# Linyou/Ced-NeRF

Measured on NVIDIA B200. Metric: train_step_rays_per_s, higher is better.
Workload: dtype f16 (MLP, tables) / f32 (marching, compositing, grads)

## Files before the change

cednerf_b200/csrc/march.cu:

```cuda
#include "common.cuh"

#define MARCH_MAX_LEVELS 8

namespace {

struct MarchArgs {
  const float* rays_o;
  const float* rays_d;
  int64_t n_rays;
  const uint32_t* occ_bits;
  const float* aabbs;
  int n_levels;
  int res;
  const float* near;
  const float* far;
  float near_const, far_const;
  float step_size, cone_angle;
  int limit;
  const uint8_t* mask;
  const float* t_sorted;
  const int64_t* t_indices;
  const uint8_t* hits;
  const int64_t* iv_starts;
  const int64_t* sm_starts;
  float* iv_vals;
  uint8_t* iv_left;
  uint8_t* iv_right;
  int64_t* iv_ray;
  float* sm_vals;
  int64_t* sm_ray;
  uint8_t* sm_valid;
  float* t_starts;
  float* t_ends;
  int64_t* ray_indices;
  int32_t* n_intervals;
  int32_t* n_samples;
  float* termination;
  float* run_t;
  int32_t* run_n;
  int32_t* n_runs;
  int run_cap;
  const int32_t* order;
  const int32_t* n_active_dev;
  const int32_t* limit_dev;
  int by_slot;
  const uint32_t* coarse;
};

__device__ __forceinline__ float clampf(float v, float lo, float hi) { return fminf(fmaxf(v, lo), hi); }
__device__ __forceinline__ int clampi(int v, int lo, int hi) { return v < lo ? lo : (v > hi ? hi : v); }
__device__ __forceinline__ float step_dt(float t, float cone, float step) { return clampf(t * cone, step, 1e10f); }

__device__ __forceinline__ void advance_to(float& t_last, float t_target, float cone, float step_size) {
  if (step_size <= 0.0f) {
    t_last = t_target;
    return;
  }
  if (cone == 0.0f && step_size <= 1e10f && t_last == t_last && t_last - t_last == 0.0f) {
    const float half = step_size * 0.5f;
    while (t_last + half < t_target) t_last += step_size;
    return;
  }
  while (!(t_last * cone >= step_size && t_target * cone < 1e10f)) {
    const float dt = step_dt(t_last, cone, step_size);
    if (t_last + dt * 0.5f >= t_target) return;
    t_last += dt;
  }
  float t = t_last;
  for (;;) {
    const float d0 = t * cone;
    const float t1 = t + d0, d1 = t1 * cone;
    const float t2 = t1 + d1, d2 = t2 * cone;
    const float t3 = t2 + d2, d3 = t3 * cone;
    const bool e0 = t + d0 * 0.5f >= t_target, e1 = t1 + d1 * 0.5f >= t_target;
    const bool e2 = t2 + d2 * 0.5f >= t_target, e3 = t3 + d3 * 0.5f >= t_target;
    if (e0 | e1 | e2 | e3) {
      t_last = e0 ? t : (e1 ? t1 : (e2 ? t2 : t3));
      return;
    }
    t = t3 + d3;
  }
}

__device__ __forceinline__ void slab(const float* o, const float* inv, const float* bx, float near, float far,
                                     float miss, float& t_min, float& t_max, bool& hit) {
  float tmin = -INFINITY, tmax = INFINITY;
#pragma unroll
  for (int a = 0; a < 3; ++a) {
    const float t1 = (bx[a] - o[a]) * inv[a];
    const float t2 = (bx[3 + a] - o[a]) * inv[a];
    tmin = fmaxf(tmin, fminf(t1, t2));
    tmax = fminf(tmax, fmaxf(t1, t2));
  }
  hit = (tmax > tmin) && (tmax > 0.0f);
  t_min = hit ? clampf(tmin, near, far) : miss;
  t_max = hit ? clampf(tmax, near, far) : miss;
}

__global__ void ray_aabb_kernel(const float* __restrict__ rays_o, const float* __restrict__ rays_d, int64_t n,
                                const float* __restrict__ aabbs, int L, float near, float far, float miss,
                                float* __restrict__ t_mins, float* __restrict__ t_maxs, uint8_t* __restrict__ hits) {
  const int64_t r = (int64_t)blockIdx.x * blockDim.x + threadIdx.x;
  if (r >= n) return;
  const float o[3] = {rays_o[3 * r], rays_o[3 * r + 1], rays_o[3 * r + 2]};
  const float inv[3] = {1.0f / rays_d[3 * r], 1.0f / rays_d[3 * r + 1], 1.0f / rays_d[3 * r + 2]};
  for (int l = 0; l < L; ++l) {
    float a, b;
    bool h;
    slab(o, inv, aabbs + 6 * l, near, far, miss, a, b, h);
    t_mins[r * L + l] = a;
    t_maxs[r * L + l] = b;
    hits[r * L + l] = (uint8_t)h;
  }
}

__device__ __forceinline__ void sort_bounds(float* v, int* id, int m) {
  for (int i = 1; i < m; ++i) {
    const float kv = v[i];
    const int ki = id[i];
    int j = i - 1;
    while (j >= 0 && v[j] > kv) {
      v[j + 1] = v[j];
      id[j + 1] = id[j];
      --j;
    }
    v[j + 1] = kv;
    id[j + 1] = ki;
  }
}

__global__ void sort_boundaries_kernel(const float* __restrict__ t_mins, const float* __restrict__ t_maxs, int64_t n,
                                       int L, float* __restrict__ t_sorted, int64_t* __restrict__ t_indices) {
  const int64_t r = (int64_t)blockIdx.x * blockDim.x + threadIdx.x;
  if (r >= n) return;
  float v[2 * MARCH_MAX_LEVELS];
  int id[2 * MARCH_MAX_LEVELS];
  const int m = 2 * L;
  for (int l = 0; l < L; ++l) {
    v[l] = t_mins[r * L + l];
    v[L + l] = t_maxs[r * L + l];
  }
  for (int i = 0; i < m; ++i) id[i] = i;
  sort_bounds(v, id, m);
  for (int i = 0; i < m; ++i) {
    t_sorted[r * m + i] = v[i];
    t_indices[r * m + i] = id[i];
  }
}

#ifndef MARCH_MIN_BLOCKS
#define MARCH_MIN_BLOCKS 6
#endif
template <bool FILL, bool COARSE = false>
__global__ void __launch_bounds__(128, MARCH_MIN_BLOCKS) march_kernel(MarchArgs a) {
  const int64_t slot = (int64_t)blockIdx.x * blockDim.x + threadIdx.x;
  if (slot >= a.n_rays) return;
  if (a.n_active_dev && slot >= (int64_t)*a.n_active_dev) {
    if (!FILL && a.n_samples) a.n_samples[slot] = 0;
    if (!FILL && a.n_runs) a.n_runs[slot] = 0;
    return;
  }
  const int64_t r = a.order ? (int64_t)a.order[slot] : slot;
  const int64_t oi = a.by_slot ? slot : r;
  const float near = a.near ? a.near[r] : a.near_const;
  const float far = a.far ? a.far[r] : a.far_const;
  if (a.mask && !a.mask[oi]) {
    if (a.n_intervals) a.n_intervals[oi] = 0;
    if (a.n_samples) a.n_samples[oi] = 0;
    if (a.termination && !(FILL && a.by_slot)) a.termination[r] = near;
    if (!FILL && a.n_runs) a.n_runs[oi] = 0;
    return;
  }
  const int L = a.n_levels, m = 2 * L, res = a.res;
  const float eps = 1e-6f;
  const float o[3] = {a.rays_o[3 * r], a.rays_o[3 * r + 1], a.rays_o[3 * r + 2]};
  const float d[3] = {a.rays_d[3 * r], a.rays_d[3 * r + 1], a.rays_d[3 * r + 2]};
  const float inv[3] = {1.0f / d[0], 1.0f / d[1], 1.0f / d[2]};
  const float fres = (float)res;
  const int64_t cells_per_level = (int64_t)res * res * res;

  float ts[2 * MARCH_MAX_LEVELS];
  int ti[2 * MARCH_MAX_LEVELS];
  bool hit[MARCH_MAX_LEVELS];
  if (a.t_sorted) {
    for (int i = 0; i < m; ++i) {
      ts[i] = a.t_sorted[r * m + i];
      ti[i] = (int)a.t_indices[r * m + i];
    }
    for (int l = 0; l < L; ++l) hit[l] = a.hits[r * L + l] != 0;
  } else {
    for (int l = 0; l < L; ++l) slab(o, inv, a.aabbs + 6 * l, -INFINITY, INFINITY, INFINITY, ts[l], ts[L + l], hit[l]);
    for (int i = 0; i < m; ++i) ti[i] = i;
    sort_bounds(ts, ti, m);
  }

  const int64_t iv_base = FILL && a.iv_starts ? a.iv_starts[oi] : 0;
  const int64_t sm_base = FILL && a.sm_starts ? a.sm_starts[oi] : 0;
  int n_iv = 0, n_sm = 0;
  float t_last = near;
  int continuous = 0;
  int runs = 0, run_len = 0;
  const int limit = a.limit_dev ? *a.limit_dev : a.limit;
  const float step_size = a.step_size, cone = a.cone_angle;

  for (int i = 0; i < m - 1; ++i) {
    const int bi = ti[i];
    const bool entering = bi < L;
    int level = bi % L;
    if (!hit[level]) continue;
    if (!entering) {
      const int bn = ti[i + 1];
      if (bn < L) continue;
      level = bn % L;
      if (!hit[level]) continue;
    }
    const float this_tmin = fmaxf(ts[i], near);
    const float this_tmax = fminf(ts[i + 1], far);
    if (this_tmin >= this_tmax) continue;

    if (!continuous) advance_to(t_last, this_tmin, cone, step_size);

    const float* bx = a.aabbs + 6 * level;
    float tdist[3], delta[3];
    int cur[3], overflow[3], stepi[3];
    const float tstart = this_tmin + eps, tend = this_tmax - eps;
#pragma unroll
    for (int ax = 0; ax < 3; ++ax) {
      const float extent = bx[3 + ax] - bx[ax];
      const float voxel = extent / fres;
      const float start = o[ax] + d[ax] * tstart;
      const float end = o[ax] + d[ax] * tend;
      int c = (int)(((start - bx[ax]) / extent) * fres);
      int f = (int)(((end - bx[ax]) / extent) * fres);
      c = clampi(c, 0, res - 1);
      f = clampi(f, 0, res - 1);
      const int start_idx = c + (d[ax] > 0.0f ? 1 : 0);
      const float tmax_a = ((bx[ax] + (((float)start_idx * voxel) - start)) * inv[ax]) + this_tmin;
      const float stepf = (d[ax] == 0.0f) ? 0.0f : (d[ax] > 0.0f ? 1.0f : -1.0f);
      tdist[ax] = (d[ax] == 0.0f) ? this_tmax : tmax_a;
      delta[ax] = (d[ax] == 0.0f) ? this_tmax : (voxel * inv[ax]) * stepf;
      stepi[ax] = (int)stepf;
      cur[ax] = c;
      overflow[ax] = f + stepi[ax];
    }

    float t_pend = 0.0f;
    int pend = 0;
    int eb0 = -1, eb1 = -1, eb2 = -1;
    auto catch_up = [&](float t_target) { advance_to(t_last, t_target, cone, step_size); };
    uint32_t cell = ((uint32_t)cur[0] * (uint32_t)res + (uint32_t)cur[1]) * (uint32_t)res + (uint32_t)cur[2] +
                    (uint32_t)level * (uint32_t)cells_per_level;
    int dcell[3] = {stepi[0] * res * res, stepi[1] * res, stepi[2]};
    asm volatile("" : "+r"(dcell[0]), "+r"(dcell[1]));
    while (limit <= 0 || n_sm < limit) {
      const float t_trav = fminf(fminf(tdist[0], fminf(tdist[1], tdist[2])), this_tmax);
      bool occupied = false;
      if (!(COARSE && (cur[0] >> 2) == eb0 && (cur[1] >> 2) == eb1 && (cur[2] >> 2) == eb2)) {
        occupied = (__ldg(a.occ_bits + (cell >> 5)) >> (cell & 31u)) & 1u;
        if (COARSE && !occupied) {
          const int cres = res >> 2;
          const int64_t cb = ((int64_t)(cur[0] >> 2) * cres + (cur[1] >> 2)) * cres + (cur[2] >> 2) +
                             (int64_t)level * cres * cres * cres;
          const bool block_occupied = (__ldg(a.coarse + (cb >> 5)) >> (cb & 31)) & 1u;
          eb0 = block_occupied ? -1 : (cur[0] >> 2);
          eb1 = cur[1] >> 2;
          eb2 = cur[2] >> 2;
        }
      }
      if (!occupied) {
        t_pend = t_trav;
        pend = 1;
        continuous = 0;
      } else {
        if (pend) {
          catch_up(t_pend);
          pend = 0;
        }
        while (limit <= 0 || n_sm < limit) {
          float t_next;
          if (step_size <= 0.0f) {
            t_next = t_trav;
          } else {
            const float dt = step_dt(t_last, cone, step_size);
            if (t_last + dt * 0.5f >= t_trav) break;
            t_next = t_last + dt;
          }
          if (FILL) {
            if (a.iv_vals) {
              const int64_t k = iv_base + n_iv;
              if (!continuous) {
                a.iv_vals[k] = t_last;
                a.iv_ray[k] = r;
                a.iv_left[k] = 1;
                a.iv_vals[k + 1] = t_next;
                a.iv_ray[k + 1] = r;
                a.iv_right[k + 1] = 1;
              } else {
                a.iv_vals[k] = t_next;
                a.iv_ray[k] = r;
                a.iv_left[k - 1] = 1;
                a.iv_right[k] = 1;
              }
            }
            const int64_t k = sm_base + n_sm;
            if (a.sm_vals) {
              a.sm_vals[k] = (t_next + t_last) * 0.5f;
              a.sm_ray[k] = r;
              a.sm_valid[k] = 1;
            }
            if (a.t_starts) {
              a.t_starts[k] = t_last;
              a.t_ends[k] = t_next;
              a.ray_indices[k] = r;
            }
          }
          if (!FILL && a.run_t) {
            if (!continuous) {
              if (runs > 0 && runs <= a.run_cap) a.run_n[oi * a.run_cap + runs - 1] = run_len;
              if (runs < a.run_cap) a.run_t[oi * a.run_cap + runs] = t_last;
              ++runs;
              run_len = 0;
            }
            ++run_len;
          }
          n_iv += continuous ? 1 : 2;
          n_sm += 1;
          continuous = 1;
          t_last = t_next;
          if (t_next >= t_trav) break;
        }
      }
      const bool s0 = tdist[0] < tdist[1] && tdist[0] < tdist[2];
      const bool s1 = !s0 && tdist[1] < tdist[2];
      const bool s2 = !s0 && !s1;
      const float n0 = tdist[0] + delta[0], n1 = tdist[1] + delta[1], n2 = tdist[2] + delta[2];
      tdist[0] = s0 ? n0 : tdist[0];
      tdist[1] = s1 ? n1 : tdist[1];
      tdist[2] = s2 ? n2 : tdist[2];
      cur[0] += s0 ? stepi[0] : 0;
      cur[1] += s1 ? stepi[1] : 0;
      cur[2] += s2 ? stepi[2] : 0;
      cell += (uint32_t)(s0 ? dcell[0] : (s1 ? dcell[1] : dcell[2]));
      const bool done = (s0 & (cur[0] == overflow[0])) | (s1 & (cur[1] == overflow[1])) | (s2 & (cur[2] == overflow[2]));
      if (done) break;
    }
    if (pend) catch_up(t_pend);
  }
  if (!FILL && a.run_t) {
    if (runs > 0 && runs <= a.run_cap) a.run_n[oi * a.run_cap + runs - 1] = run_len;
    a.n_runs[oi] = runs;
  }
  if (a.n_intervals) a.n_intervals[oi] = n_iv;
  if (a.n_samples) a.n_samples[oi] = n_sm;
  const bool refilled = a.by_slot && !FILL && runs > a.run_cap;
  if (a.termination && !refilled) a.termination[r] = t_last;
}

__global__ void __launch_bounds__(128)
march_fill_runs_kernel(int64_t n_rays, const int64_t* __restrict__ sm_starts, const float* __restrict__ run_t,
                       const int32_t* __restrict__ run_n, const int32_t* __restrict__ n_runs, int run_cap,
                       float step_size, float cone, float* __restrict__ t_starts, float* __restrict__ t_ends,
                       int64_t* __restrict__ ray_indices, uint8_t* __restrict__ overflow,
                       const int32_t* __restrict__ capped_counts, const int32_t* __restrict__ slot_ray = nullptr,
                       const int32_t* __restrict__ n_active_dev = nullptr) {
  const int64_t r = (int64_t)blockIdx.x * blockDim.x + threadIdx.x;
  if (r >= n_rays) return;
  if (n_active_dev && r >= (int64_t)*n_active_dev) {
    overflow[r] = 0;
    return;
  }
  const int64_t ray_id = slot_ray ? (int64_t)slot_ray[r] : r;
  const int runs = n_runs[r];
  bool over = runs > run_cap;
  int64_t k = sm_starts[r];
  const int64_t k_end = capped_counts ? sm_starts[r + 1] : INT64_MAX;
  if (capped_counts && over && k_end - k != (int64_t)capped_counts[r]) {
    for (; k < k_end; ++k) t_starts[k] = 0.0f, t_ends[k] = 0.0f, ray_indices[k] = ray_id;
    over = false;
    overflow[r] = 0;
    return;
  }
  overflow[r] = (uint8_t)over;
  if (over) return;
  auto next = [&](float t) { return (step_size <= 0.0f) ? t : t + step_dt(t, cone, step_size); };
  for (int j = 0; j < runs; ++j) {
    float t = run_t[r * run_cap + j];
    int cnt = run_n[r * run_cap + j];
    if ((int64_t)cnt > k_end - k) cnt = (int)(k_end - k);
    int i = 0;
    for (; i < cnt && (k & 3); ++i, ++k) {
      const float t_next = next(t);
      t_starts[k] = t, t_ends[k] = t_next, ray_indices[k] = ray_id;
      t = t_next;
    }
    for (; i + 4 <= cnt; i += 4, k += 4) {
      const float a1 = next(t), a2 = next(a1), a3 = next(a2), a4 = next(a3);
      *reinterpret_cast<float4*>(t_starts + k) = make_float4(t, a1, a2, a3);
      *reinterpret_cast<float4*>(t_ends + k) = make_float4(a1, a2, a3, a4);
      const longlong2 rr = make_longlong2((long long)ray_id, (long long)ray_id);
      *reinterpret_cast<longlong2*>(ray_indices + k) = rr;
      *reinterpret_cast<longlong2*>(ray_indices + k + 2) = rr;
      t = a4;
    }
    for (; i < cnt; ++i, ++k) {
      const float t_next = next(t);
      t_starts[k] = t, t_ends[k] = t_next, ray_indices[k] = ray_id;
      t = t_next;
    }
  }
}

__global__ void pack_bits_kernel(const uint8_t* __restrict__ bin, int64_t n_cells, uint32_t* __restrict__ bits) {
  const int64_t i = (int64_t)blockIdx.x * blockDim.x + threadIdx.x;
  const bool b = i < n_cells && bin[i] != 0;
  const unsigned w = __ballot_sync(0xffffffffu, b);
  if ((threadIdx.x & 31) == 0 && i < n_cells) bits[i >> 5] = w;
}

__global__ void occ_threshold_kernel(const float* __restrict__ occs, int64_t n_cells, const float* __restrict__ thre,
                                     uint8_t* __restrict__ bin, uint32_t* __restrict__ bits) {
  const int64_t i = (int64_t)blockIdx.x * blockDim.x + threadIdx.x;
// ... 132 lines not shown
      totals[0] = t < capacity ? t : capacity;
      totals[1] = t;
    }
  }
  __syncthreads();
  int64_t off = excl_s + local;
#pragma unroll
  for (int k = 0; k < SCAN_ITEMS; ++k) {
    if (base + k < n) offsets[base + k] = off < capacity ? off : capacity;
    off += c[k];
  }
}

}

CEDNERF_EXPORT int cednerf_ray_aabb_intersect(const float* rays_o, const float* rays_d, int64_t n_rays,
                                              const float* aabbs, int n_levels, float near_plane, float far_plane,
                                              float miss_value, float* t_mins, float* t_maxs, uint8_t* hits,
                                              void* stream) {
  CEDNERF_REQUIRE(n_rays >= 0 && n_levels >= 1, "bad sizes");
  if (n_rays == 0) return 0;
  ray_aabb_kernel<<<cednerf_blocks(n_rays, 256), 256, 0, (cudaStream_t)stream>>>(
      rays_o, rays_d, n_rays, aabbs, n_levels, near_plane, far_plane, miss_value, t_mins, t_maxs, hits);
  return cednerf_check_launch("cednerf_ray_aabb_intersect");
}

CEDNERF_EXPORT int cednerf_sort_boundaries(const float* t_mins, const float* t_maxs, int64_t n_rays, int n_levels,
                                           float* t_sorted, int64_t* t_indices, void* stream) {
  CEDNERF_REQUIRE(n_rays >= 0 && n_levels >= 1 && n_levels <= MARCH_MAX_LEVELS, "bad sizes (levels <= 8)");
  if (n_rays == 0) return 0;
  sort_boundaries_kernel<<<cednerf_blocks(n_rays, 256), 256, 0, (cudaStream_t)stream>>>(t_mins, t_maxs, n_rays,
                                                                                       n_levels, t_sorted, t_indices);
  return cednerf_check_launch("cednerf_sort_boundaries");
}

CEDNERF_EXPORT int cednerf_occ_pack_bits(const uint8_t* binaries, int64_t n_cells, uint32_t* bits, void* stream) {
  CEDNERF_REQUIRE(n_cells > 0, "empty grid");
  pack_bits_kernel<<<cednerf_blocks(n_cells, 256), 256, 0, (cudaStream_t)stream>>>(binaries, n_cells, bits);
  return cednerf_check_launch("cednerf_occ_pack_bits");
}

CEDNERF_EXPORT int cednerf_occ_threshold_pack(const float* occs, int64_t n_cells, const float* threshold_dev,
                                              uint8_t* binaries, uint32_t* bits, void* stream) {
  CEDNERF_REQUIRE(n_cells > 0 && (n_cells % 32) == 0, "cell count must be a multiple of 32");
  occ_threshold_kernel<<<cednerf_blocks(n_cells, 256), 256, 0, (cudaStream_t)stream>>>(occs, n_cells, threshold_dev,
                                                                                      binaries, bits);
  return cednerf_check_launch("cednerf_occ_threshold_pack");
}

namespace {

__global__ void __launch_bounds__(256) occ_mark_invisible_kernel(const float* __restrict__ K, int n_K,
                                                                 const float* __restrict__ c2w, int n_cams, int c2w_rows,
                                                                 const float* __restrict__ aabbs, int res,
                                                                 int64_t cells_per_level, int64_t n_cells, float width,
                                                                 float height, float near, float* __restrict__ occs) {
  __shared__ float cam[64][21];
  const int64_t cell = (int64_t)blockIdx.x * blockDim.x + threadIdx.x;
  const bool active = cell < n_cells;
  float xw[3] = {0.f, 0.f, 0.f};
  if (active) {
    const int level = (int)(cell / cells_per_level);
    const int64_t c = cell - (int64_t)level * cells_per_level;
    const int coord[3] = {(int)(c / ((int64_t)res * res)), (int)((c / res) % res), (int)(c % res)};
    const float* bx = aabbs + 6 * level;
#pragma unroll
    for (int k = 0; k < 3; ++k) {
      const float x01 = __fdiv_rn((float)coord[k], (float)(res - 1));
      xw[k] = __fadd_rn(bx[k], __fmul_rn(x01, __fsub_rn(bx[3 + k], bx[k])));
    }
  }
  bool covered = false, too_near = false;
  for (int c0 = 0; c0 < n_cams; c0 += 64) {
    const int nc = n_cams - c0 < 64 ? n_cams - c0 : 64;
    __syncthreads();
    for (int q = threadIdx.x; q < nc; q += blockDim.x) {
      const float* m = c2w + (int64_t)(c0 + q) * c2w_rows * 4;
      const float* k = K + (n_K == 1 ? 0 : (int64_t)(c0 + q) * 9);
      float* d = cam[q];
#pragma unroll
      for (int i = 0; i < 3; ++i) {
#pragma unroll
        for (int j = 0; j < 3; ++j) d[3 * i + j] = m[4 * j + i];
        d[9 + i] = -__fadd_rn(__fadd_rn(__fmul_rn(m[i], m[3]), __fmul_rn(m[4 + i], m[7])), __fmul_rn(m[8 + i], m[11]));
      }
#pragma unroll
      for (int j = 0; j < 9; ++j) d[12 + j] = k[j];
    }
    __syncthreads();
    if (active) {
      for (int q = 0; q < nc; ++q) {
        const float* d = cam[q];
        float xc[3], uvd[3];
#pragma unroll
        for (int i = 0; i < 3; ++i)
          xc[i] = __fadd_rn(__fadd_rn(__fadd_rn(__fmul_rn(d[3 * i], xw[0]), __fmul_rn(d[3 * i + 1], xw[1])),
                                      __fmul_rn(d[3 * i + 2], xw[2])),
                            d[9 + i]);
#pragma unroll
        for (int i = 0; i < 3; ++i)
          uvd[i] = __fadd_rn(__fadd_rn(__fmul_rn(d[12 + 3 * i], xc[0]), __fmul_rn(d[12 + 3 * i + 1], xc[1])),
                             __fmul_rn(d[12 + 3 * i + 2], xc[2]));
        const float u = __fdiv_rn(uvd[0], uvd[2]), v = __fdiv_rn(uvd[1], uvd[2]);
        const bool in_image = uvd[2] >= 0.f && u >= 0.f && u < width && v >= 0.f && v < height;
        covered = covered || (uvd[2] >= near && in_image);
        too_near = too_near || (uvd[2] < near && in_image);
      }
    }
  }
  if (active) occs[cell] = (covered && !too_near) ? 0.f : -1.f;
}

}

CEDNERF_EXPORT int cednerf_occ_mark_invisible(const float* K, int n_K, const float* c2w, int n_cams, int c2w_rows,
                                              const float* aabbs, int n_levels, int resolution, int width, int height,
                                              float near_plane, float* occs, void* stream) {
  CEDNERF_REQUIRE(K && c2w && aabbs && occs, "null argument");
  CEDNERF_REQUIRE(n_cams >= 1 && (n_K == 1 || n_K == n_cams) && (c2w_rows == 3 || c2w_rows == 4), "bad camera arrays");
  CEDNERF_REQUIRE(n_levels >= 1 && resolution >= 2, "bad grid");
  const int64_t cpl = (int64_t)resolution * resolution * resolution, n_cells = cpl * n_levels;
  occ_mark_invisible_kernel<<<cednerf_blocks(n_cells, 256), 256, 0, (cudaStream_t)stream>>>(
      K, n_K, c2w, n_cams, c2w_rows, aabbs, resolution, cpl, n_cells, (float)width, (float)height, near_plane, occs);
  return cednerf_check_launch("cednerf_occ_mark_invisible");
}

namespace {

__global__ void ray_coherence_keys_kernel(const float* __restrict__ rays_d, int64_t n, int32_t* __restrict__ keys) {
  const int64_t r = (int64_t)blockIdx.x * blockDim.x + threadIdx.x;
  if (r >= n) return;
  const float x = rays_d[3 * r], y = rays_d[3 * r + 1], z = rays_d[3 * r + 2];
  const float inv = 1.0f / fmaxf(fabsf(x) + fabsf(y) + fabsf(z), 1e-20f);
  float u = x * inv, v = y * inv;
  if (z < 0.0f) {
    const float fu = (1.0f - fabsf(v)) * (u >= 0.0f ? 1.0f : -1.0f), fv = (1.0f - fabsf(u)) * (v >= 0.0f ? 1.0f : -1.0f);
    u = fu, v = fv;
  }
  uint32_t qu = (uint32_t)fminf(fmaxf((u * 0.5f + 0.5f) * 1023.0f, 0.0f), 1023.0f);
  uint32_t qv = (uint32_t)fminf(fmaxf((v * 0.5f + 0.5f) * 1023.0f, 0.0f), 1023.0f);
  auto spread = [](uint32_t b) {
    b = (b | (b << 8)) & 0x00ff00ffu;
    b = (b | (b << 4)) & 0x0f0f0f0fu;
    b = (b | (b << 2)) & 0x33333333u;
    b = (b | (b << 1)) & 0x55555555u;
    return b;
  };
  keys[r] = (int32_t)(spread(qu) | (spread(qv) << 1));
}

__global__ void occ_coarsen_kernel(const uint32_t* __restrict__ bits, int n_levels, int res, uint32_t* __restrict__ coarse) {
  const int cres = res >> 2;
  const int64_t per_level = (int64_t)cres * cres * cres, total = per_level * n_levels;
  const int64_t i = (int64_t)blockIdx.x * blockDim.x + threadIdx.x;
  if (i * 32 >= total) return;
  uint32_t w = 0u;
  for (int j = 0; j < 32; ++j) {
    const int64_t cb = i * 32 + j;
    if (cb >= total) break;
    const int level = (int)(cb / per_level);
    const int64_t r = cb - level * per_level;
    const int bz = (int)(r % cres), by = (int)((r / cres) % cres), bx = (int)(r / ((int64_t)cres * cres));
    bool any = false;
    for (int dx = 0; dx < 4 && !any; ++dx)
      for (int dy = 0; dy < 4 && !any; ++dy) {
        const int64_t c0 = ((int64_t)(4 * bx + dx) * res + (4 * by + dy)) * res + 4 * bz + (int64_t)level * res * res * res;
        for (int dz = 0; dz < 4; ++dz) {
          const int64_t c = c0 + dz;
          any = any || ((bits[c >> 5] >> (c & 31)) & 1u);
        }
      }
    if (any) w |= 1u << j;
  }
  coarse[i] = w;
}

#define ORDER_BINS 16384
__global__ void order_hist_kernel(const int32_t* __restrict__ keys, int64_t n, uint32_t* __restrict__ hist) {
  const int64_t i = (int64_t)blockIdx.x * blockDim.x + threadIdx.x;
  if (i < n) atomicAdd(hist + (((uint32_t)keys[i]) >> 6), 1u);
}
__global__ void __launch_bounds__(1024) order_scan_kernel(uint32_t* __restrict__ hist) {
  __shared__ uint32_t warp_tot[32];
  uint32_t v[16], s = 0;
#pragma unroll
  for (int k = 0; k < 16; ++k) v[k] = hist[threadIdx.x * 16 + k], s += v[k];
  uint32_t incl = s;
  const int lane = threadIdx.x & 31, warp = threadIdx.x >> 5;
#pragma unroll
  for (int o = 1; o < 32; o <<= 1) {
    const uint32_t t = __shfl_up_sync(0xffffffffu, incl, o);
    if (lane >= o) incl += t;
  }
  if (lane == 31) warp_tot[warp] = incl;
  __syncthreads();
  if (warp == 0) {
    uint32_t w = warp_tot[lane], wi = w;
#pragma unroll
    for (int o = 1; o < 32; o <<= 1) {
      const uint32_t t = __shfl_up_sync(0xffffffffu, wi, o);
      if (lane >= o) wi += t;
    }
    warp_tot[lane] = wi - w;
  }
  __syncthreads();
  uint32_t off = warp_tot[warp] + incl - s;
#pragma unroll
  for (int k = 0; k < 16; ++k) hist[threadIdx.x * 16 + k] = off, off += v[k];
}
__global__ void order_scatter_kernel(const int32_t* __restrict__ keys, int64_t n, uint32_t* __restrict__ cursor,
                                     int32_t* __restrict__ order) {
  const int64_t i = (int64_t)blockIdx.x * blockDim.x + threadIdx.x;
  if (i < n) order[atomicAdd(cursor + (((uint32_t)keys[i]) >> 6), 1u)] = (int32_t)i;
}

}

CEDNERF_EXPORT int cednerf_ray_coherence_order(const int32_t* keys, int64_t n_rays, int32_t* order, void* workspace,
                                               void* stream) {
  CEDNERF_REQUIRE(n_rays >= 0 && n_rays < (1ll << 31) && keys && order && workspace, "bad arguments");
  if (n_rays == 0) return 0;
  cudaStream_t st = (cudaStream_t)stream;
  uint32_t* hist = (uint32_t*)workspace;
  cudaMemsetAsync(hist, 0, ORDER_BINS * sizeof(uint32_t), st);
  order_hist_kernel<<<cednerf_blocks(n_rays, 256), 256, 0, st>>>(keys, n_rays, hist);
  order_scan_kernel<<<1, 1024, 0, st>>>(hist);
  order_scatter_kernel<<<cednerf_blocks(n_rays, 256), 256, 0, st>>>(keys, n_rays, hist, order);
  return cednerf_check_launch("cednerf_ray_coherence_order", 3);
}

CEDNERF_EXPORT int cednerf_occ_coarsen(const uint32_t* occ_bits, int n_levels, int resolution, uint32_t* coarse, void* stream) {
  CEDNERF_REQUIRE(occ_bits && coarse && n_levels >= 1 && resolution >= 4 && resolution % 4 == 0, "bad arguments");
  const int cres = resolution / 4;
  const int64_t words = ((int64_t)cres * cres * cres * n_levels + 31) / 32;
  occ_coarsen_kernel<<<cednerf_blocks(words, 128), 128, 0, (cudaStream_t)stream>>>(occ_bits, n_levels, resolution, coarse);
  return cednerf_check_launch("cednerf_occ_coarsen");
}

CEDNERF_EXPORT int cednerf_ray_coherence_keys(const float* rays_d, int64_t n_rays, int32_t* keys, void* stream) {
  CEDNERF_REQUIRE(n_rays >= 0 && rays_d && keys, "bad arguments");
  if (n_rays == 0) return 0;
  ray_coherence_keys_kernel<<<cednerf_blocks(n_rays, 256), 256, 0, (cudaStream_t)stream>>>(rays_d, n_rays, keys);
  return cednerf_check_launch("cednerf_ray_coherence_keys");
}

CEDNERF_EXPORT int cednerf_march(int fill, const float* rays_o, const float* rays_d, int64_t n_rays,
                                 const uint32_t* occ_bits, const float* aabbs, int n_levels, int resolution,
                                 const float* near_planes, const float* far_planes, float near_const, float far_const,
                                 float step_size, float cone_angle, int steps_limit, const uint8_t* rays_mask,
                                 const float* t_sorted, const int64_t* t_indices, const uint8_t* hits,
                                 const int64_t* iv_starts, const int64_t* sm_starts, float* iv_vals, uint8_t* iv_left,
                                 uint8_t* iv_right, int64_t* iv_ray, float* sm_vals, int64_t* sm_ray,
                                 uint8_t* sm_valid, float* t_starts, float* t_ends, int64_t* ray_indices,
                                 int32_t* n_intervals, int32_t* n_samples, float* termination, float* run_t,
                                 int32_t* run_n, int32_t* n_runs, int run_cap, const int32_t* ray_order,
                                 const uint32_t* occ_coarse, void* stream) {
  CEDNERF_REQUIRE(!run_t || (!fill && run_n && n_runs && run_cap > 0 && step_size > 0.0f),
                  "run recording: count pass, positive step size");
  CEDNERF_REQUIRE((int64_t)n_levels * resolution * resolution * resolution < (1ll << 31), "occupancy grid too large");
  CEDNERF_REQUIRE(n_rays >= 0 && n_levels >= 1 && n_levels <= MARCH_MAX_LEVELS && resolution >= 1,
                  "bad sizes (levels <= 8)");
  CEDNERF_REQUIRE((t_sorted == nullptr) == (t_indices == nullptr) && (t_sorted == nullptr) == (hits == nullptr),
                  "t_sorted, t_indices and hits go together");
  CEDNERF_REQUIRE(!fill || ((!t_starts && !sm_vals) || sm_starts) , "fill pass needs sm_starts");
  CEDNERF_REQUIRE(!fill || !iv_vals || iv_starts, "fill pass needs iv_starts");
  CEDNERF_REQUIRE(!t_starts || (t_ends && ray_indices), "packed outputs go together");
  if (n_rays == 0) return 0;
  MarchArgs a{rays_o, rays_d, n_rays, occ_bits, aabbs, n_levels, resolution, near_planes, far_planes, near_const,
              far_const, step_size, cone_angle, steps_limit, rays_mask, t_sorted, t_indices, hits, iv_starts,
              sm_starts, iv_vals, iv_left, iv_right, iv_ray, sm_vals, sm_ray, sm_valid, t_starts, t_ends, ray_indices,
              n_intervals, n_samples, termination, run_t, run_n, n_runs, run_cap, ray_order, nullptr, nullptr, 0,
              (resolution % 4 == 0) ? occ_coarse : nullptr};
  const unsigned grid = cednerf_blocks(n_rays, 128);
  if (a.coarse) {
    if (fill) march_kernel<true, true><<<grid, 128, 0, (cudaStream_t)stream>>>(a);
    else march_kernel<false, true><<<grid, 128, 0, (cudaStream_t)stream>>>(a);
  } else {
    if (fill) march_kernel<true><<<grid, 128, 0, (cudaStream_t)stream>>>(a);
    else march_kernel<false><<<grid, 128, 0, (cudaStream_t)stream>>>(a);
  }
  return cednerf_check_launch("cednerf_march");
}

CEDNERF_EXPORT int cednerf_march_fill_runs(int64_t n_rays, const int64_t* sm_starts, const float* run_t,
                                           const int32_t* run_n, const int32_t* n_runs, int run_cap, float step_size,
                                           float cone_angle, float* t_starts, float* t_ends, int64_t* ray_indices,
                                           uint8_t* overflow, void* stream) {
  CEDNERF_REQUIRE(n_rays >= 0 && run_cap > 0 && step_size > 0.0f, "bad arguments");
  CEDNERF_REQUIRE((((uintptr_t)t_starts | (uintptr_t)t_ends | (uintptr_t)ray_indices) & 15) == 0,
                  "packed outputs must be 16-byte aligned");
  if (n_rays == 0) return 0;
  march_fill_runs_kernel<<<cednerf_blocks(n_rays, 128), 128, 0, (cudaStream_t)stream>>>(
      n_rays, sm_starts, run_t, run_n, n_runs, run_cap, step_size, cone_angle, t_starts, t_ends, ray_indices, overflow,
      nullptr);
  return cednerf_check_launch("cednerf_march_fill_runs");
}

CEDNERF_EXPORT int cednerf_march_fill_runs_capped(int64_t n_rays, const int64_t* offsets, const int32_t* n_samples,
                                                  const float* run_t, const int32_t* run_n, const int32_t* n_runs,
                                                  int run_cap, float step_size, float cone_angle, float* t_starts,
                                                  float* t_ends, int64_t* ray_indices, uint8_t* overflow, void* stream) {
  CEDNERF_REQUIRE(n_rays >= 0 && run_cap > 0 && step_size > 0.0f && offsets && n_samples, "bad arguments");
  CEDNERF_REQUIRE((((uintptr_t)t_starts | (uintptr_t)t_ends | (uintptr_t)ray_indices) & 15) == 0,
                  "packed outputs must be 16-byte aligned");
  if (n_rays == 0) return 0;
  march_fill_runs_kernel<<<cednerf_blocks(n_rays, 128), 128, 0, (cudaStream_t)stream>>>(
      n_rays, offsets, run_t, run_n, n_runs, run_cap, step_size, cone_angle, t_starts, t_ends, ray_indices, overflow,
      n_samples);
  return cednerf_check_launch("cednerf_march_fill_runs_capped");
}

CEDNERF_EXPORT int64_t cednerf_scan_workspace_bytes(int64_t n) {
  const int64_t tiles = (n + SCAN_TILE - 1) / SCAN_TILE;
  return 8 * (tiles + 1);
}

CEDNERF_EXPORT int cednerf_exclusive_scan(const int32_t* counts, int64_t n, int64_t* starts, int64_t* packed_info,
                                          int64_t* total, void* workspace, void* stream) {
  CEDNERF_REQUIRE(n >= 0 && workspace, "bad arguments");
  cudaStream_t st = (cudaStream_t)stream;
  if (n == 0) {
    if (total) cudaMemsetAsync(total, 0, 8, st);
    return 0;
  }
  const int64_t tiles = (n + SCAN_TILE - 1) / SCAN_TILE;
  int64_t* tile_sums = (int64_t*)workspace;
  scan_tile_sums_kernel<<<(unsigned)tiles, SCAN_THREADS, 0, st>>>(counts, n, tile_sums);
  scan_tile_offsets_kernel<<<1, SCAN_THREADS, 0, st>>>(tile_sums, tiles, total);
  scan_apply_kernel<<<(unsigned)tiles, SCAN_THREADS, 0, st>>>(counts, n, tile_sums, starts, packed_info);
  return cednerf_check_launch("cednerf_exclusive_scan", 3);
}

CEDNERF_EXPORT int cednerf_exclusive_scan_capped(const int32_t* counts, int64_t n, int64_t capacity, int64_t* offsets,
                                                 int64_t* totals, void* workspace, void* stream) {
  CEDNERF_REQUIRE(n >= 0 && capacity >= 0 && offsets && totals && workspace, "bad arguments");
  cudaStream_t st = (cudaStream_t)stream;
  if (n == 0) {
    cudaMemsetAsync(offsets, 0, 8, st);
    cudaMemsetAsync(totals, 0, 16, st);
    return 0;
  }
  const int64_t tiles = (n + SCAN_TILE - 1) / SCAN_TILE;
  cudaMemsetAsync(workspace, 0, 8 * (size_t)(tiles + 1), st);
  scan_capped_onepass_kernel<<<(unsigned)tiles, SCAN_THREADS, 0, st>>>(counts, n, capacity, offsets, totals,
                                                                       (unsigned long long*)workspace);
  return cednerf_check_launch("cednerf_exclusive_scan_capped", 1);
}

namespace {
__global__ void render_round_begin_kernel(int32_t* __restrict__ state, int64_t n_rays, int max_samples, int min_samples,
                                          const int64_t* __restrict__ prev_totals, int64_t* __restrict__ total) {
  cednerf_round_begin(state, n_rays, max_samples, min_samples, prev_totals, total);
}
}

CEDNERF_EXPORT int cednerf_render_round_begin(int32_t* state, int64_t n_rays, int max_samples, int min_samples,
                                              const int64_t* prev_totals, int64_t* total, void* stream) {
  CEDNERF_REQUIRE(state && n_rays >= 0 && max_samples > 0 && min_samples > 0, "bad arguments");
  render_round_begin_kernel<<<1, 1, 0, (cudaStream_t)stream>>>(state, n_rays, max_samples, min_samples, prev_totals, total);
  return cednerf_check_launch("cednerf_render_round_begin");
}

CEDNERF_EXPORT int cednerf_march_round(int fill, const float* rays_o, const float* rays_d, int64_t n_bound,
                                       const uint32_t* occ_bits, const float* aabbs, int n_levels, int resolution,
                                       float* near_term, float far_const, float step_size, float cone_angle,
                                       const float* t_sorted, const int64_t* t_indices, const uint8_t* hits,
                                       const int32_t* alive, const int32_t* state, const uint8_t* slot_mask,
                                       const int64_t* offsets, float* t_starts, float* t_ends, int64_t* ray_indices,
                                       int32_t* n_samples, float* run_t, int32_t* run_n, int32_t* n_runs, int run_cap,
                                       const uint32_t* occ_coarse, void* stream) {
  CEDNERF_REQUIRE((int64_t)n_levels * resolution * resolution * resolution < (1ll << 31), "occupancy grid too large");
  CEDNERF_REQUIRE(n_bound >= 0 && n_levels >= 1 && n_levels <= MARCH_MAX_LEVELS && resolution >= 1 && alive && state &&
                      near_term && t_sorted && t_indices && hits,
                  "bad arguments");
  CEDNERF_REQUIRE(fill ? (slot_mask && offsets && t_starts && t_ends && ray_indices)
                       : (n_samples && run_t && run_n && n_runs && run_cap > 0 && step_size > 0.0f),
                  "count pass: counts and runs; fill pass: mask, offsets and packed outputs");
  if (n_bound == 0) return 0;
  MarchArgs a{};
  a.rays_o = rays_o, a.rays_d = rays_d, a.n_rays = n_bound, a.occ_bits = occ_bits, a.aabbs = aabbs;
  a.n_levels = n_levels, a.res = resolution, a.near = near_term, a.far = nullptr, a.near_const = 0.0f, a.far_const = far_const;
  a.step_size = step_size, a.cone_angle = cone_angle, a.limit = 0, a.mask = fill ? slot_mask : nullptr;
  a.t_sorted = t_sorted, a.t_indices = t_indices, a.hits = hits;
  a.sm_starts = offsets, a.t_starts = t_starts, a.t_ends = t_ends, a.ray_indices = ray_indices;
  a.n_samples = fill ? nullptr : n_samples, a.termination = near_term;
  a.run_t = fill ? nullptr : run_t, a.run_n = fill ? nullptr : run_n, a.n_runs = fill ? nullptr : n_runs, a.run_cap = run_cap;
  a.order = alive, a.n_active_dev = state, a.limit_dev = state + 1, a.by_slot = 1;
  a.coarse = (resolution % 4 == 0) ? occ_coarse : nullptr;
// ... 26 lines not shown
```

cednerf_b200/ops.py:

```python
from __future__ import annotations

import ctypes
import math
from typing import List, Optional, Sequence, Tuple

import torch

from . import _lib
from ._lib import FieldDesc, GridLevels, MlpDesc, call, ptr, stream

F32, F16, I64, I32, U8 = torch.float32, torch.float16, torch.int64, torch.int32, torch.uint8


def _f32c(t: torch.Tensor) -> torch.Tensor:
    _lib.check_device()
    if not t.is_cuda:
        raise RuntimeError("cednerf_b200 ops need CUDA tensors (no CPU fallback)")
    return t.detach().to(F32).contiguous()


def ray_aabb_intersect(rays_o, rays_d, aabbs, near_plane=-math.inf, far_plane=math.inf, miss_value=math.inf):
    o, d, bx = _f32c(rays_o), _f32c(rays_d), _f32c(aabbs)
    n, nl = o.shape[0], bx.shape[0]
    t_mins = torch.empty(n, nl, device=o.device)
    t_maxs = torch.empty(n, nl, device=o.device)
    hits = torch.empty(n, nl, dtype=torch.bool, device=o.device)
    call("cednerf_ray_aabb_intersect", ptr(o), ptr(d), n, ptr(bx), nl, near_plane, far_plane, miss_value,
         ptr(t_mins), ptr(t_maxs), ptr(hits), stream())
    return t_mins, t_maxs, hits


def sort_boundaries(t_mins, t_maxs):
    a, b = _f32c(t_mins), _f32c(t_maxs)
    n, nl = a.shape
    t_sorted = torch.empty(n, 2 * nl, device=a.device)
    t_indices = torch.empty(n, 2 * nl, dtype=I64, device=a.device)
    call("cednerf_sort_boundaries", ptr(a), ptr(b), n, nl, ptr(t_sorted), ptr(t_indices), stream())
    return t_sorted, t_indices


def pack_occupancy(binaries: torch.Tensor) -> torch.Tensor:
    _lib.check_device()
    b = binaries.detach().contiguous()
    if b.dtype != torch.bool and b.dtype != U8:
        b = b.to(torch.bool)
    n_cells = b.numel()
    bits = torch.empty((n_cells + 31) // 32, dtype=I32, device=b.device)
    call("cednerf_occ_pack_bits", ptr(b), n_cells, ptr(bits), stream())
    return bits


def occ_threshold_pack(occs: torch.Tensor, threshold: torch.Tensor, binaries: torch.Tensor, bits: torch.Tensor):
    call("cednerf_occ_threshold_pack", ptr(occs), occs.numel(), ptr(threshold), ptr(binaries), ptr(bits), stream())


def exclusive_scan(counts: torch.Tensor, want_packed: bool = True):
    n = counts.numel()
    dev = counts.device
    starts = torch.empty(n, dtype=I64, device=dev)
    packed = torch.empty(n, 2, dtype=I64, device=dev) if want_packed else None
    total = torch.empty(1, dtype=I64, device=dev)
    ws = torch.empty(max(int(_lib.load().cednerf_scan_workspace_bytes(n)) // 8, 1), dtype=I64, device=dev)
    call("cednerf_exclusive_scan", ptr(counts), n, ptr(starts), ptr(packed), ptr(total), ptr(ws), stream())
    return starts, packed, total


def counts_of(t: Optional[torch.Tensor]):
    return getattr(t, "_cednerf_counts", None) if t is not None else None


def exclusive_scan_capped(counts: torch.Tensor, capacity: int):
    n, dev = counts.numel(), counts.device
    offsets = torch.empty(n + 1, dtype=I64, device=dev)
    totals = torch.empty(2, dtype=I64, device=dev)
    ws = torch.empty(max(int(_lib.load().cednerf_scan_workspace_bytes(n)) // 8, 1), dtype=I64, device=dev)
    call("cednerf_exclusive_scan_capped", ptr(counts), n, int(capacity), ptr(offsets), ptr(totals), ptr(ws), stream())
    return offsets, totals


def occupancy_coarse(bits: torch.Tensor, n_levels: int, res: int):
    if res % 4 or bits is None:
        return None
    hit = getattr(bits, "_cednerf_coarse", None)
    if hit is not None and hit[0] == bits._version:
        return hit[1]
    words = (n_levels * (res // 4) ** 3 + 31) // 32
    coarse = torch.empty(words, dtype=I32, device=bits.device)
    call("cednerf_occ_coarsen", ptr(bits), n_levels, res, ptr(coarse), stream())
    bits._cednerf_coarse = (bits._version, coarse)
    return coarse


class MarchInputs:

    def __init__(self, rays_o, rays_d, occ_bits, aabbs, resolution, near_planes=None, far_planes=None,
                 near_const=0.0, far_const=math.inf, step_size=1e-3, cone_angle=0.0, limit=-1, rays_mask=None,
                 t_sorted=None, t_indices=None, hits=None):
        self.o, self.d = _f32c(rays_o), _f32c(rays_d)
        self.bits, self.aabbs = occ_bits, _f32c(aabbs)
        self.n, self.nl, self.res = self.o.shape[0], self.aabbs.shape[0], int(resolution)
        self.near = None if near_planes is None else _f32c(near_planes)
        self.far = None if far_planes is None else _f32c(far_planes)
        self.near_const, self.far_const = float(near_const), float(far_const)
        self.step, self.cone, self.limit = float(step_size), float(cone_angle), int(limit)
        self.mask = None if rays_mask is None else rays_mask.detach().to(torch.bool).contiguous()
        self.t_sorted = None if t_sorted is None else _f32c(t_sorted)
        self.t_indices = None if t_indices is None else t_indices.detach().to(I64).contiguous()
        self.hits = None if hits is None else hits.detach().to(torch.bool).contiguous()
        self.order = None
        self.coarse = None

    def sort_for_coherence(self):
        keys = torch.empty(self.n, dtype=I32, device=self.o.device)
        call("cednerf_ray_coherence_keys", ptr(self.d), self.n, ptr(keys), stream())
        self.order = torch.empty(self.n, dtype=I32, device=self.o.device)
        ws = torch.empty(16384, dtype=I32, device=self.o.device)
        call("cednerf_ray_coherence_order", ptr(keys), self.n, ptr(self.order), ptr(ws), stream())

    def _common(self, fill):
        return (fill, ptr(self.o), ptr(self.d), self.n, ptr(self.bits), ptr(self.aabbs), self.nl, self.res,
                ptr(self.near), ptr(self.far), self.near_const, self.far_const, self.step, self.cone, self.limit,
                ptr(self.mask), ptr(self.t_sorted), ptr(self.t_indices), ptr(self.hits))

    RUN_CAP = 16

    def count(self, record_runs: bool = False):
        dev = self.o.device
        n_iv = torch.empty(self.n, dtype=I32, device=dev)
        n_sm = torch.empty(self.n, dtype=I32, device=dev)
        term = torch.empty(self.n, device=dev)
        self.runs = None
        if record_runs and self.step > 0:
            self.runs = (torch.empty(self.n, self.RUN_CAP, device=dev), torch.empty(self.n, self.RUN_CAP, dtype=I32, device=dev),
                         torch.empty(self.n, dtype=I32, device=dev))
        rt, rn, nr = self.runs if self.runs is not None else (None, None, None)
        call("cednerf_march", *self._common(0), None, None, None, None, None, None, None, None, None, None, None,
             None, ptr(n_iv), ptr(n_sm), ptr(term), ptr(rt), ptr(rn), ptr(nr), self.RUN_CAP if rt is not None else 0,
             ptr(self.order), ptr(self.coarse), stream())
        return n_iv, n_sm, term

    def fill_packed_from_runs(self, sm_starts, total):
        dev = self.o.device
        t0 = _sempty(total, device=dev)
        t1 = _sempty(total, device=dev)
        ridx = _sempty(total, dtype=I64, device=dev)
        overflow = torch.empty(self.n, dtype=torch.bool, device=dev)
        rt, rn, nr = self.runs
        call("cednerf_march_fill_runs", self.n, ptr(sm_starts), ptr(rt), ptr(rn), ptr(nr), self.RUN_CAP, self.step,
             self.cone, ptr(t0), ptr(t1), ptr(ridx), ptr(overflow), stream())
        user_mask, self.mask = self.mask, overflow
        call("cednerf_march", *self._common(1), None, ptr(sm_starts), None, None, None, None, None, None, None,
             ptr(t0), ptr(t1), ptr(ridx), None, None, None, None, None, None, 0, None, ptr(self.coarse), stream())
        self.mask = user_mask
        return ridx, t0, t1

    def fill_packed_capped(self, offsets, n_sm, capacity):
        dev = self.o.device
        t0 = torch.empty(capacity, device=dev)
        t1 = torch.empty(capacity, device=dev)
        ridx = torch.empty(capacity, dtype=I64, device=dev)
        overflow = torch.empty(self.n, dtype=torch.bool, device=dev)
        rt, rn, nr = self.runs
        call("cednerf_march_fill_runs_capped", self.n, ptr(offsets), ptr(n_sm), ptr(rt), ptr(rn), ptr(nr), self.RUN_CAP,
             self.step, self.cone, ptr(t0), ptr(t1), ptr(ridx), ptr(overflow), stream())
        user_mask, self.mask = self.mask, overflow
        call("cednerf_march", *self._common(1), None, ptr(offsets), None, None, None, None, None, None, None,
             ptr(t0), ptr(t1), ptr(ridx), None, None, None, None, None, None, 0, None, ptr(self.coarse), stream())
        self.mask = user_mask
        return ridx, t0, t1

    def fill_packed(self, sm_starts, total):
        dev = self.o.device
        t0 = _sempty(total, device=dev)
        t1 = _sempty(total, device=dev)
        ridx = _sempty(total, dtype=I64, device=dev)
        term = torch.empty(self.n, device=dev)
        call("cednerf_march", *self._common(1), None, ptr(sm_starts), None, None, None, None, None, None, None,
             ptr(t0), ptr(t1), ptr(ridx), None, None, ptr(term), None, None, None, 0, None, ptr(self.coarse), stream())
        return ridx, t0, t1, term

    def fill_nerfacc(self, iv_starts, sm_starts, n_iv_total, n_sm_total):
        dev = self.o.device
        iv_vals = torch.zeros(n_iv_total, device=dev)
        iv_left = torch.zeros(n_iv_total, dtype=torch.bool, device=dev)
        iv_right = torch.zeros(n_iv_total, dtype=torch.bool, device=dev)
        iv_ray = torch.zeros(n_iv_total, dtype=I64, device=dev)
        sm_vals = torch.zeros(n_sm_total, device=dev)
        sm_ray = torch.zeros(n_sm_total, dtype=I64, device=dev)
        sm_valid = torch.zeros(n_sm_total, dtype=torch.bool, device=dev)
        n_iv = torch.empty(self.n, dtype=I32, device=dev)
        n_sm = torch.empty(self.n, dtype=I32, device=dev)
        term = torch.empty(self.n, device=dev)
        call("cednerf_march", *self._common(1), ptr(iv_starts), ptr(sm_starts), ptr(iv_vals), ptr(iv_left),
             ptr(iv_right), ptr(iv_ray), ptr(sm_vals), ptr(sm_ray), ptr(sm_valid), None, None, None, ptr(n_iv),
             ptr(n_sm), ptr(term), None, None, None, 0, None, ptr(self.coarse), stream())
        return (iv_vals, iv_left, iv_right, iv_ray), (sm_vals, sm_ray, sm_valid), n_iv, n_sm, term


def grid_levels(n_levels: int, base_resolution: float, log_per_level_scale: float, max_params: int):
    import numpy as np

    if n_levels > _lib.MAX_LEVELS:
        raise ValueError(f"at most {_lib.MAX_LEVELS} levels")
    g = GridLevels()
    g.n_levels = n_levels
    off = 0
    info = []
    for l in range(n_levels):
        s = float(base_resolution) * math.exp(float(l) * log_per_level_scale) - 1.0
        res = int(math.ceil(s)) + 1
        full = res ** 3
        size = min(int(max_params), (full + 7) // 8 * 8)
        if full > size and size & (size - 1):
            raise ValueError(f"hashed level {l}: max_params must be a power of two, got {max_params}")
        g.scale[l] = float(np.float32(s))
        g.res[l], g.size[l], g.offset[l], g.hashed[l] = res, size, off, int(full > size)
        info.append((float(np.float32(s)), res, size, off, full > size))
        off += size
    return g, off, info


def cast_f16(src: torch.Tensor) -> torch.Tensor:
    s = _f32c(src).view(-1)
    dst = torch.empty(s.numel(), dtype=F16, device=s.device)
    call("cednerf_cast_f32_to_f16", ptr(s), ptr(dst), s.numel(), stream())
    return dst


def _cap(n: int) -> int:
    return (int(n) + 32767) // 32768 * 32768


_capacities: List[int] = []


def _sticky_capacity(n: int) -> int:
    n = int(n)
    if n < 65536:
        return n
    best = 0
    for c in _capacities:
        if n <= c <= n * 13 // 10 and (best == 0 or c < best):
            best = c
    if best == 0:
        best = (n * 11 // 10 + 65535) // 65536 * 65536
        _capacities.append(best)
        if len(_capacities) > 64:
            del _capacities[0]
    return best


def _sempty(n: int, *tail, dtype=None, device=None) -> torch.Tensor:
    cap = _sticky_capacity(n)
    t = torch.empty((cap,) + tuple(tail), dtype=dtype, device=device)
    return t if cap == n else t[:n]


_param_epoch = 0


def note_parameter_gradient():
    global _param_epoch
    _param_epoch += 1
# ... 455 lines not shown
```

Baseline: 54.28 million.

## Skip empty 4x4x4 occupancy blocks in one step and enable coarse grid by default

When a coarse 4x4x4 block is empty, the ray marcher now computes the block exit analytically and jumps the DDA state (tdist, cur, cell) past the whole block, where before it stepped cell by cell through it. The coarse grid is now built unconditionally in MarchInputs, so this path runs by default. The coarsen kernel is rewritten to give one block per thread, read 4-bit nibbles and pack the results with a warp ballot. The aim is fewer DDA iterations and memory loads in empty space. The costs are an extra coarse-grid build on every construction and an occ_word load issued before the coarse check, and the exit arithmetic must match the stepwise traversal exactly.

```diff
diff --git a/cednerf_b200/csrc/march.cu b/cednerf_b200/csrc/march.cu
--- a/cednerf_b200/csrc/march.cu
+++ b/cednerf_b200/csrc/march.cu
@@ -1,4 +1,5 @@
 #include "common.cuh"
+#include "march_block.cuh"
 
 #define MARCH_MAX_LEVELS 8
 
@@ -246,27 +247,31 @@
 
     float t_pend = 0.0f;
     int pend = 0;
-    int eb0 = -1, eb1 = -1, eb2 = -1;
     auto catch_up = [&](float t_target) { advance_to(t_last, t_target, cone, step_size); };
     uint32_t cell = ((uint32_t)cur[0] * (uint32_t)res + (uint32_t)cur[1]) * (uint32_t)res + (uint32_t)cur[2] +
                     (uint32_t)level * (uint32_t)cells_per_level;
     int dcell[3] = {stepi[0] * res * res, stepi[1] * res, stepi[2]};
     asm volatile("" : "+r"(dcell[0]), "+r"(dcell[1]));
+    const int cres = res >> 2;
+    const uint32_t cb_level = (uint32_t)level * (uint32_t)(cres * cres * cres);
+    const bool blockable = COARSE && march_blockable(tdist, delta, cur, stepi, overflow);
     while (limit <= 0 || n_sm < limit) {
-      const float t_trav = fminf(fminf(tdist[0], fminf(tdist[1], tdist[2])), this_tmax);
-      bool occupied = false;
-      if (!(COARSE && (cur[0] >> 2) == eb0 && (cur[1] >> 2) == eb1 && (cur[2] >> 2) == eb2)) {
-        occupied = (__ldg(a.occ_bits + (cell >> 5)) >> (cell & 31u)) & 1u;
-        if (COARSE && !occupied) {
-          const int cres = res >> 2;
-          const int64_t cb = ((int64_t)(cur[0] >> 2) * cres + (cur[1] >> 2)) * cres + (cur[2] >> 2) +
-                             (int64_t)level * cres * cres * cres;
-          const bool block_occupied = (__ldg(a.coarse + (cb >> 5)) >> (cb & 31)) & 1u;
-          eb0 = block_occupied ? -1 : (cur[0] >> 2);
-          eb1 = cur[1] >> 2;
-          eb2 = cur[2] >> 2;
+      const uint32_t occ_word = __ldg(a.occ_bits + (cell >> 5));
+      if (COARSE && blockable) {
+        const uint32_t cb = ((uint32_t)(cur[0] >> 2) * (uint32_t)cres + (uint32_t)(cur[1] >> 2)) * (uint32_t)cres +
+                            (uint32_t)(cur[2] >> 2) + cb_level;
+        if (!((__ldg(a.coarse + (cb >> 5)) >> (cb & 31u)) & 1u)) {
+          int nx[3];
+          const bool done = march_block_exit(tdist, delta, cur, stepi, overflow, this_tmax, t_pend, nx);
+          pend = 1;
+          continuous = 0;
+          cell += (uint32_t)(nx[0] * dcell[0] + nx[1] * dcell[1] + nx[2] * dcell[2]);
+          if (done) break;
+          continue;
         }
       }
+      const float t_trav = fminf(fminf(tdist[0], fminf(tdist[1], tdist[2])), this_tmax);
+      const bool occupied = (occ_word >> (cell & 31u)) & 1u;
       if (!occupied) {
         t_pend = t_trav;
         pend = 1;
@@ -705,27 +710,24 @@
 __global__ void occ_coarsen_kernel(const uint32_t* __restrict__ bits, int n_levels, int res, uint32_t* __restrict__ coarse) {
   const int cres = res >> 2;
   const int64_t per_level = (int64_t)cres * cres * cres, total = per_level * n_levels;
-  const int64_t i = (int64_t)blockIdx.x * blockDim.x + threadIdx.x;
-  if (i * 32 >= total) return;
-  uint32_t w = 0u;
-  for (int j = 0; j < 32; ++j) {
-    const int64_t cb = i * 32 + j;
-    if (cb >= total) break;
+  const int64_t cb = (int64_t)blockIdx.x * blockDim.x + threadIdx.x;
+  bool any = false;
+  if (cb < total) {
     const int level = (int)(cb / per_level);
     const int64_t r = cb - level * per_level;
     const int bz = (int)(r % cres), by = (int)((r / cres) % cres), bx = (int)(r / ((int64_t)cres * cres));
-    bool any = false;
-    for (int dx = 0; dx < 4 && !any; ++dx)
-      for (int dy = 0; dy < 4 && !any; ++dy) {
+    uint32_t acc = 0u;
+#pragma unroll
+    for (int dx = 0; dx < 4; ++dx)
+#pragma unroll
+      for (int dy = 0; dy < 4; ++dy) {
         const int64_t c0 = ((int64_t)(4 * bx + dx) * res + (4 * by + dy)) * res + 4 * bz + (int64_t)level * res * res * res;
-        for (int dz = 0; dz < 4; ++dz) {
-          const int64_t c = c0 + dz;
-          any = any || ((bits[c >> 5] >> (c & 31)) & 1u);
-        }
+        acc |= (__ldg(bits + (c0 >> 5)) >> (c0 & 31)) & 0xfu;
       }
-    if (any) w |= 1u << j;
-  }
-  coarse[i] = w;
+    any = acc != 0u;
+  }
+  const unsigned w = __ballot_sync(0xffffffffu, any);
+  if ((threadIdx.x & 31) == 0 && cb < total) coarse[cb >> 5] = w;
 }
 
 #define ORDER_BINS 16384
@@ -785,8 +787,8 @@
 CEDNERF_EXPORT int cednerf_occ_coarsen(const uint32_t* occ_bits, int n_levels, int resolution, uint32_t* coarse, void* stream) {
   CEDNERF_REQUIRE(occ_bits && coarse && n_levels >= 1 && resolution >= 4 && resolution % 4 == 0, "bad arguments");
   const int cres = resolution / 4;
-  const int64_t words = ((int64_t)cres * cres * cres * n_levels + 31) / 32;
-  occ_coarsen_kernel<<<cednerf_blocks(words, 128), 128, 0, (cudaStream_t)stream>>>(occ_bits, n_levels, resolution, coarse);
+  const int64_t blocks = (int64_t)cres * cres * cres * n_levels;
+  occ_coarsen_kernel<<<cednerf_blocks(blocks, 128), 128, 0, (cudaStream_t)stream>>>(occ_bits, n_levels, resolution, coarse);
   return cednerf_check_launch("cednerf_occ_coarsen");
 }
 
diff --git a/cednerf_b200/csrc/march_block.cuh b/cednerf_b200/csrc/march_block.cuh
--- /dev/null
+++ b/cednerf_b200/csrc/march_block.cuh
@@ -0,0 +1,68 @@
+#pragma once
+
+#if defined(__CUDACC__)
+#define MARCH_HD __host__ __device__ __forceinline__
+#else
+#include <math.h>
+#define MARCH_HD inline
+#endif
+
+MARCH_HD bool march_blockable(const float tdist[3], const float delta[3], const int cur[3], const int stepi[3],
+                              const int overflow[3]) {
+  bool ok = true;
+#pragma unroll
+  for (int ax = 0; ax < 3; ++ax)
+    ok = ok && (stepi[ax] == 0 ? (cur[ax] == overflow[ax] && tdist[ax] == tdist[ax])
+                               : (delta[ax] >= 0.0f && tdist[ax] > -INFINITY));
+  return ok;
+}
+
+MARCH_HD bool march_block_exit(float tdist[3], const float delta[3], int cur[3], const int stepi[3],
+                               const int overflow[3], float this_tmax, float& t_pend, int n[3]) {
+  int e[3];
+  float c[3];
+#pragma unroll
+  for (int ax = 0; ax < 3; ++ax) {
+    const int in_block = cur[ax] & 3;
+    const int face = stepi[ax] > 0 ? 4 - in_block : (stepi[ax] < 0 ? in_block + 1 : 1);
+    const int to_end = (overflow[ax] - cur[ax]) * stepi[ax];
+    e[ax] = (to_end >= 1 && to_end < face) ? to_end : face;
+    float p = tdist[ax];
+    c[ax] = p;
+#pragma unroll
+    for (int j = 1; j < 4; ++j) {
+      p = p + delta[ax];
+      c[ax] = j < e[ax] ? p : c[ax];
+    }
+  }
+  const bool x0 = c[0] < c[1] && c[0] < c[2];
+  const bool x1 = !x0 && c[1] < c[2];
+  const int X = x0 ? 0 : (x1 ? 1 : 2);
+  const float tx = x0 ? c[0] : (x1 ? c[1] : c[2]);
+  float h[3];
+#pragma unroll
+  for (int ax = 0; ax < 3; ++ax) {
+    float p = tdist[ax];
+    int k = 0;
+    h[ax] = p;
+#pragma unroll
+    for (int j = 0; j < 3; ++j) {
+      const bool before = j < e[ax] - 1 && (ax == X || p < tx || (p == tx && ax > X));
+      p = p + delta[ax];
+      k = before ? j + 1 : k;
+      h[ax] = before ? p : h[ax];
+    }
+    n[ax] = k;
+  }
+  t_pend = fminf(fminf(h[0], fminf(h[1], h[2])), this_tmax);
+  bool done = false;
+#pragma unroll
+  for (int ax = 0; ax < 3; ++ax) {
+    const bool s = ax == X;
+    tdist[ax] = s ? h[ax] + delta[ax] : h[ax];
+    n[ax] += s ? 1 : 0;
+    cur[ax] += n[ax] * stepi[ax];
+    done = done || (s && cur[ax] == overflow[ax]);
+  }
+  return done;
+}
diff --git a/cednerf_b200/ops.py b/cednerf_b200/ops.py
--- a/cednerf_b200/ops.py
+++ b/cednerf_b200/ops.py
@@ -108,7 +108,7 @@
         self.t_indices = None if t_indices is None else t_indices.detach().to(I64).contiguous()
         self.hits = None if hits is None else hits.detach().to(torch.bool).contiguous()
         self.order = None
-        self.coarse = None
+        self.coarse = occupancy_coarse(occ_bits, self.nl, self.res)
 
     def sort_for_coherence(self):
         keys = torch.empty(self.n, dtype=I32, device=self.o.device)
```

Result: slower. 52.90 million, median of 6 (-2.5%).
